# wh-xu/Hyper-Gen

Measured on AMD Instinct MI355X. Metric: genomes/sec sketch (k=21,s=1500,D=4096), higher is better.
Workload: dtype u64

## Files before the change

### hyper-gen_amd/__init__.py

```python
import ctypes as C
import os
import threading
import subprocess

import numpy as np

_HERE = os.path.dirname(os.path.abspath(__file__))
LIB_PATH = (os.environ.get("HYPERGEN_LIB") or None) or os.path.join(_HERE, "libhypergen_hip.so")
CLI_PATH = os.path.join(_HERE, "hyper-gen")

LAYOUT_SCALAR, LAYOUT_AVX2 = 0, 1
GATHER_PEER, GATHER_RCCL = 0, 1
ANI_MASH, ANI_CONTAINMENT, ANI_MAX_CONTAINMENT = 0, 1, 2
PAIRS_MASH, PAIRS_CONTAINMENT, PAIRS_MAX_CONTAINMENT, PAIRS_CONTAINMENT_REF = 1, 2, 4, 8
PAIRS_EMPTY = 0xFFFFFFFF
NORM_ACGT, NORM_U2T = 0, 1
(OK, ERR_INVALID, ERR_NO_DEVICE, ERR_HIP, ERR_OOM, ERR_CAPACITY, ERR_UNSUPPORTED, ERR_IO,
 ERR_INEXACT) = range(9)


T_NAMES = ("kmer", "sort", "encode", "dist_prep", "dist")
T_COUNT = len(T_NAMES)


# ... 5 lines not shown

class SketchParams(C.Structure):
    _fields_ = [("ksize", C.c_uint32), ("canonical", C.c_uint32), ("scaled", C.c_uint64),
                ("seed", C.c_uint64), ("hv_d", C.c_uint32), ("hv_layout", C.c_uint32),
                ("norm_mode", C.c_uint32), ("min_count", C.c_uint32)]


class AniHit(C.Structure):
    _fields_ = [("ref_idx", C.c_uint32), ("qry_idx", C.c_uint32), ("ani", C.c_float)]


ANI_HIT_DTYPE = np.dtype([("ref_idx", "<u4"), ("qry_idx", "<u4"), ("ani", "<f4")])
HAM_HIT_DTYPE = np.dtype([("ref_idx", "<u4"), ("qry_idx", "<u4"), ("dist", "<u4")])


class FileSketch(C.Structure):
    _fields_ = [("ksize", C.c_uint8), ("canonical", C.c_uint8), ("hv_quant_bits", C.c_uint8),
                ("pad", C.c_uint8), ("hv_norm_2", C.c_int32), ("scaled", C.c_uint64),
                ("seed", C.c_uint64), ("hv_d", C.c_uint64), ("file_str", C.c_char_p),
                ("hv", C.POINTER(C.c_int16)), ("hv_len", C.c_uint64)]


EXPORTS = [
    "hg_status_str", "hg_last_error", "hg_version", "hg_ctx_create", "hg_ctx_destroy",
    "hg_ctx_set_stream", "hg_ctx_reset_stream", "hg_ctx_sync", "hg_ctx_sketch_step_counts", "hg_sketch_plan_describe", "hg_logf_dev", "hg_ani_from_dots_dev", "hg_device_count", "hg_dev_alloc", "hg_dev_free",
    "hg_copy_h2d", "hg_copy_d2h", "hg_sketch_params_default", "hg_kmer_hash_sample",
    "hg_kmer_hash_sample_min_count",
    "hg_hv_encode", "hg_sketch_batch_dev", "hg_sketch_batch", "hg_dist_full", "hg_dist_full_dev",
    "hg_dist", "hg_dist_dev", "hg_sort_ani_hits", "hg_hv_quant_bits", "hg_hv_pack", "hg_hv_packed_bytes",
    "hg_hv_unpack", "hg_sketch_file_write", "hg_sketch_file_read", "hg_sketch_file_count",
    "hg_sketch_file_get", "hg_sketch_file_free", "hg_read_merge_seq", "hg_read_merge_seq_into", "hg_free",
    "hg_synth_genomes_dev", "hg_ctx_enable_timing", "hg_ctx_timings", "hg_ctx_last_kernel",
    "hg_hv_binarize_dev", "hg_hamming_full_dev", "hg_hamming_search_dev",
    "hg_ctx_set_debug", "hg_read_fastx_into", "hg_dist_block_dev", "hg_hamming_search_block_dev",
    "hg_multi_create", "hg_multi_destroy", "hg_multi_size", "hg_multi_ctx", "hg_multi_last_error", "hg_shard_range",
    "hg_multi_peer_report", "hg_multi_set_gather", "hg_multi_gather_mode", "hg_multi_gather_report",
    "hg_sketch_batch_multi", "hg_dist_multi", "hg_dist_multi_dev", "hg_hamming_search_multi",
    "hg_sort_ani_hits_dev", "hg_sort_ani_hits_staged", "hg_topk_per_query_dev", "hg_ctx_last_dist_path",
    "hg_ctx_last_hamming_path", "hg_read_fastx_pinned", "hg_pinned_free",
    "hg_sketch_stream_open", "hg_sketch_stream_push", "hg_sketch_stream_pop", "hg_sketch_stream_finish",
    "hg_sketch_stream_last_error", "hg_sketch_stream_close", "hg_sketch_stream_stats", "hg_device_numa_node", "hg_bind_thread_to_numa_node", "hg_dist_tile_order",
    "hg_sketch_stream_push_packed", "hg_pack2_size", "hg_pack2", "hg_unpack2_dev",
    "hg_sketch_stream_try_push", "hg_sketch_stream_max_pending",
    "hg_sketch_batch_dev_packed", "hg_pack2_batch_dev", "hg_pack2_dev",
    "hg_pack2s_size", "hg_pack2s", "hg_sketch_stream_push_packed_sparse",
    "hg_dist_ops_row_bytes", "hg_dist_ops_meta_bytes", "hg_dist_ops_padded_rows", "hg_dist_prep_ops_dev", "hg_dist_block_ops_dev",
    "hg_hv_packed_bytes_naive", "hg_hv_pack_naive", "hg_hv_unpack_naive", "hg_hv_payload_layout", "hg_hv_unpack_batch_dev",
    "hg_sketch_file_read_image", "hg_sketch_file_image", "hg_sketch_file_payload_offset",
    "hg_cluster_init_dev", "hg_cluster_add_hits_dev", "hg_cluster_finish_dev", "hg_cluster_dev", "hg_cluster",
    "hg_cluster_greedy_hits_dev", "hg_cluster_greedy_dev", "hg_cluster_greedy", "hg_ctx_cluster_greedy_rounds",
    "hg_cluster_setcover_hits_dev", "hg_cluster_setcover_dev", "hg_cluster_setcover", "hg_ctx_cluster_setcover_rounds",
    "hg_cluster_tree_hits_dev", "hg_cluster_tree_dev", "hg_cluster_tree", "hg_ctx_cluster_tree_rounds",
    "hg_cluster_average_matrix_dev", "hg_cluster_average_dev", "hg_cluster_average", "hg_ctx_cluster_average_rounds",
    "hg_cluster_complete_matrix_dev", "hg_cluster_complete_dev", "hg_cluster_complete", "hg_ctx_cluster_complete_rounds",
    "hg_cluster_stats_matrix_dev", "hg_cluster_stats_dev", "hg_cluster_stats",
    "hg_nj_matrix_dev", "hg_nj_dev", "hg_nj", "hg_nj_newick",
    "hg_ctx_set_ani_metric", "hg_ctx_ani_metric", "hg_multi_set_ani_metric",
    "hg_search_topk_dev", "hg_search_topk_block_dev", "hg_search_topk", "hg_search_topk_merge", "hg_search_topk_multi_dev",
    "hg_ani_pairs_dev", "hg_ani_pairs",
]
SEARCH_TOPK_MAX = 64
CLUSTER_AVERAGE_MAX_N = 65536
CLUSTER_COMPLETE_MAX_N = 65536
STATS_NONE = 0xFFFFFFFF
NJ_MAX_N = 65536
NJ_FRAC_BITS = 15
NJ_JOIN_DTYPE = np.dtype([("a", "<u4"), ("b", "<u4"), ("len_a", "<i8"), ("len_b", "<i8")])


class NodeStat(C.Structure):
    _fields_ = [("within_sum", C.c_uint64), ("within_min", C.c_uint32), ("within_min_idx", C.c_uint32),
                ("outside_max", C.c_uint32), ("outside_max_idx", C.c_uint32)]
# ... 67 lines not shown
        "hg_copy_d2h": (C.c_int, [vp, vp, vp, sz]),
        "hg_sketch_params_default": (None, [C.POINTER(SketchParams)]),
        "hg_kmer_hash_sample": (C.c_int, [vp, vp, sz, C.c_uint32, C.c_uint64, C.c_uint64, C.c_int,
                                          C.c_uint32, vp, sz, C.POINTER(sz)]),
        "hg_kmer_hash_sample_min_count": (C.c_int, [vp, vp, sz, C.c_uint32, C.c_uint64, C.c_uint64, C.c_int,
                                                    C.c_uint32, C.c_uint32, vp, sz, C.POINTER(sz)]),
        "hg_hv_encode": (C.c_int, [vp, vp, sz, C.c_uint32, C.c_uint32, vp, C.POINTER(C.c_int32)]),
        "hg_sketch_batch_dev": (C.c_int, [vp, vp, vp, vp, sz, C.POINTER(SketchParams), vp, vp, vp]),
        "hg_sketch_batch": (C.c_int, [vp, C.POINTER(vp), C.POINTER(sz), sz, C.POINTER(SketchParams),
                                      vp, vp, vp]),
        "hg_dist_full": (C.c_int, [vp, vp, vp, sz, vp, vp, sz, C.c_uint32, C.c_uint32, vp]),
        "hg_dist_full_dev": (C.c_int, [vp, vp, vp, sz, vp, vp, sz, C.c_uint32, C.c_uint32, vp]),
        "hg_ani_pairs_dev": (C.c_int, [vp, vp, vp, sz, vp, vp, sz, C.c_uint32, C.c_uint32, vp, sz, C.c_uint32, vp, vp]),
        "hg_ani_pairs": (C.c_int, [vp, vp, vp, sz, vp, vp, sz, C.c_uint32, C.c_uint32, vp, sz, C.c_uint32, vp, vp]),
        "hg_dist": (C.c_int, [vp, vp, vp, sz, vp, vp, sz, C.c_uint32, C.c_uint32, C.c_int, C.c_float,
                              vp, sz, C.POINTER(sz)]),
        "hg_dist_dev": (C.c_int, [vp, vp, vp, sz, vp, vp, sz, C.c_uint32, C.c_uint32, C.c_int,
                                  C.c_float, vp, sz, C.POINTER(sz)]),
        "hg_sort_ani_hits": (None, [vp, sz, sz, C.c_int]),
        "hg_hv_quant_bits": (C.c_uint32, [vp, C.c_uint32]),
        "hg_hv_pack": (C.c_int, [vp, C.c_uint32, C.c_uint32, vp]),
        "hg_hv_packed_bytes": (sz, [C.c_uint32, C.c_uint32]),
        "hg_hv_unpack": (C.c_int, [vp, C.c_uint32, C.c_uint32, vp]),
        "hg_sketch_file_write": (C.c_int, [C.c_char_p, C.POINTER(FileSketch), sz]),
        "hg_sketch_file_read": (C.c_int, [C.c_char_p, C.POINTER(vp)]),
        "hg_sketch_file_count": (sz, [vp]),
        "hg_sketch_file_get": (C.POINTER(FileSketch), [vp, sz]),
        "hg_sketch_file_free": (None, [vp]),
        "hg_read_merge_seq": (C.c_int, [C.c_char_p, C.POINTER(vp), C.POINTER(sz)]),
        "hg_read_merge_seq_into": (C.c_int, [C.c_char_p, C.POINTER(vp), C.POINTER(sz), C.POINTER(sz)]),
        "hg_read_fastx_into": (C.c_int, [C.c_char_p, C.c_uint32, C.POINTER(vp), C.POINTER(sz), C.POINTER(sz)]),
        "hg_ctx_set_debug": (C.c_int, [vp, C.c_char_p, C.c_char_p]),
        "hg_free": (None, [vp]),
        "hg_read_fastx_pinned": (C.c_int, [C.c_char_p, C.c_uint32, C.POINTER(vp), C.POINTER(sz), C.POINTER(sz)]),
        "hg_pinned_free": (None, [vp]),
        "hg_device_numa_node": (C.c_int, [C.c_int]),
        "hg_bind_thread_to_numa_node": (C.c_int, [C.c_int, C.c_uint]),
        "hg_dist_tile_order": (C.c_int, [C.c_uint32, C.c_uint32, C.c_uint32, C.c_uint32, C.c_int, C.c_int, C.c_uint64, C.c_uint64,
                                         C.c_void_p, C.c_size_t, C.POINTER(C.c_size_t)]),
        "hg_sketch_stream_open": (C.c_int, [C.POINTER(C.c_int), C.c_int, C.POINTER(SketchParams), C.POINTER(vp)]),
        "hg_sketch_stream_push": (C.c_int, [vp, vp, sz, C.c_uint64]),
        "hg_sketch_stream_pop": (C.c_int, [vp, C.POINTER(C.c_uint64), vp, C.POINTER(C.c_int32), C.POINTER(C.c_uint32),
                                           C.POINTER(C.c_int)]),
        "hg_sketch_stream_push_packed": (C.c_int, [vp, vp, sz, C.c_uint64]),
        "hg_sketch_stream_try_push": (C.c_int, [vp, vp, sz, C.c_uint64, C.c_int]),
        "hg_sketch_stream_max_pending": (sz, [vp]),
        "hg_pack2_size": (sz, [sz]),
        "hg_pack2": (C.c_int, [vp, sz, C.c_uint32, vp]),
        "hg_unpack2_dev": (C.c_int, [vp, vp, sz, vp]),
        "hg_sketch_batch_dev_packed": (C.c_int, [vp, vp, vp, vp, sz, C.POINTER(SketchParams), vp, vp, vp]),
        "hg_pack2_batch_dev": (C.c_int, [vp, vp, vp, vp, sz, C.c_uint32, vp, vp]),
        "hg_pack2_dev": (C.c_int, [vp, vp, sz, C.c_uint32, vp]),
        "hg_dist_ops_row_bytes": (sz, [C.c_uint32]),
        "hg_dist_ops_meta_bytes": (sz, []),
        "hg_dist_ops_padded_rows": (sz, [sz]),
        "hg_dist_prep_ops_dev": (C.c_int, [vp, vp, sz, C.c_uint32, vp, vp, vp]),
        "hg_dist_block_ops_dev": (C.c_int, [vp, vp, vp, vp, sz, sz, vp, vp, sz, vp, vp, sz, sz, C.c_uint32, C.c_uint32, C.c_int,
                                            C.c_float, vp, sz, C.POINTER(sz)]),
        "hg_pack2s_size": (sz, [sz, sz]),
        "hg_pack2s": (C.c_int, [vp, sz, C.c_uint32, vp, sz, C.POINTER(sz)]),
        "hg_sketch_stream_push_packed_sparse": (C.c_int, [vp, vp, sz, sz, C.c_uint64]),
        "hg_sketch_stream_finish": (C.c_int, [vp]),
        "hg_sketch_stream_last_error": (C.c_char_p, [vp]),
        "hg_sketch_stream_close": (None, [vp]),
        "hg_sketch_stream_stats": (C.c_int, [vp, C.c_int, C.POINTER(C.c_double)]),
        "hg_ctx_last_dist_path": (C.c_int, [vp]),
        "hg_ctx_set_ani_metric": (C.c_int, [vp, C.c_int]),
# ... 1257 lines not shown
```

### hyper-gen_amd/csrc/hg_api_sketch.hip

```cpp
#include <algorithm>
#include <atomic>
#include <cctype>
#include <chrono>
#include <cstdio>
#include <cstring>
#include <functional>
#include <memory>
#include <sched.h>
#include <string>
#include <thread>
#include <vector>

#include "hg_host.h"
#include "hg_hostfed_layout.h"

#include "hg_sketch.h"

static hg_status sketch_batch_dev_impl(hg_ctx *c, const uint8_t *d_seq, const uint64_t *offsets, const uint64_t *lens, size_t n,
                                       const hg_sketch_params *p, int16_t *d_hv, int32_t *d_norm2, uint32_t *d_nhash, bool packed,
                                       const uint64_t *mask_offs = nullptr) {
  if (!c) return HG_ERR_INVALID;
  hg_status s = hg_check_sketch_params(c, p);
  if (s != HG_OK) return s;
  if (n == 0) return HG_OK;
// ... 51 lines not shown
  if (((uintptr_t)d_seq & 3) || ((uintptr_t)d_blob & 15)) return hg_fail(c, HG_ERR_INVALID, "hg_pack2_dev: d_seq must be 4-byte, d_blob 16-byte aligned");
  const uint64_t zero = 0, len = n_bps;
  return hg_pack2_batch_dev(c, d_seq, &zero, &len, 1, norm_mode, d_blob, &zero);
}

extern "C" int hg_device_numa_node(int device_id) {
  char bus[64] = {0};
  if (hipDeviceGetPCIBusId(bus, (int)sizeof bus, device_id) != hipSuccess) return -1;
  for (char *q = bus; *q; ++q) *q = (char)std::tolower((unsigned char)*q);
  const std::string path = std::string("/sys/bus/pci/devices/") + bus + "/numa_node";
  FILE *f = std::fopen(path.c_str(), "r");
  if (!f) return -1;
  int node = -1;
  if (std::fscanf(f, "%d", &node) != 1) node = -1;
  std::fclose(f);
  return node;
}

namespace {
bool grow_pinned(uint8_t *&buf, size_t &cap, size_t need, size_t keep, void *) {
  if (need <= cap) return true;
  const size_t want = ((need + need / 8) + ((size_t)1 << 20) - 1) & ~(((size_t)1 << 20) - 1);
  void *nb = nullptr;
  if (hipHostMalloc(&nb, want, hipHostMallocPortable) != hipSuccess || !nb) return false;
  if (buf && keep) std::memcpy(nb, buf, std::min(keep, cap));
  if (buf) (void)hipHostFree(buf);
  buf = static_cast<uint8_t *>(nb), cap = want;
  return true;
}
}

extern "C" hg_status hg_read_fastx_pinned(const char *path, uint32_t mode, uint8_t **buf, size_t *cap, size_t *n_bps) {
  return hg_read_fastx_impl(path, mode, buf, cap, n_bps, grow_pinned, nullptr);
}

extern "C" void hg_pinned_free(void *p) {
  if (p) (void)hipHostFree(p);
}

static unsigned host_threads() {
  unsigned n = std::thread::hardware_concurrency();
  cpu_set_t set;
  if (sched_getaffinity(0, sizeof set, &set) == 0) n = std::min<unsigned>(n ? n : 1u, (unsigned)CPU_COUNT(&set));
  return std::max(1u, std::min(n, 16u));
}

static std::atomic<int> g_hostfed_calls{0};
namespace {
struct HostfedCall {
  int others;
  HostfedCall() : others(g_hostfed_calls.fetch_add(1)) {}
  ~HostfedCall() { g_hostfed_calls.fetch_sub(1); }
};
}
static bool host_pinned(const void *p) {
  hipPointerAttribute_t a;
  if (hipPointerGetAttributes(&a, p) != hipSuccess) {
    (void)hipGetLastError();
    return false;
  }
  return a.type == hipMemoryTypeHost;
}
namespace {
constexpr double HG_LINK_BYTES_PER_S = 50e9;
struct PackState {
  std::atomic<uint64_t> rate{0};
// ... 361 lines not shown
```

### hyper-gen_amd/csrc/hg_cli.cpp

```cpp
#include <fcntl.h>
#include <glob.h>
#include <sched.h>
#include <unistd.h>
#include <sys/stat.h>

#include <algorithm>
#include <atomic>
#include <bitset>
#include <cerrno>
#include <chrono>
#include <condition_variable>
#include <cstdarg>
#include <cstdio>
#include <cstdlib>
#include <cstring>
#include <ctime>
#include <deque>
#include <initializer_list>
#include <map>
#include <mutex>
#include <string>
#include <thread>
#include <utility>
#include <vector>

#include "../../include/hypergen.h"
#include "../../include/hypergen_aa.h"
#include "../../include/hypergen_tx.h"

namespace {

void logline(const char *lvl, const std::string &msg) {
  char ts[32];
  std::time_t t = std::time(nullptr);
  std::strftime(ts, sizeof ts, "%Y-%m-%d-%H:%M:%S", std::localtime(&t));
  std::printf("%s [%s] - %s\n", ts, lvl, msg.c_str());
  std::fflush(stdout);
}

bool debug_log() {
  static const bool on = [] {
    const char *e = std::getenv("RUST_LOG");
    return e && std::strstr(e, "debug") != nullptr;
  }();
  return on;
}
double now_s() { return std::chrono::duration<double>(std::chrono::steady_clock::now().time_since_epoch()).count(); }
void debugf(const char *fmt, ...) __attribute__((format(printf, 1, 2)));
void debugf(const char *fmt, ...) {
  if (!debug_log()) return;
  char buf[512];
  va_list ap;
  va_start(ap, fmt);
  std::vsnprintf(buf, sizeof buf, fmt, ap);
  va_end(ap);
  logline("DEBUG", buf);
}

[[noreturn]] void die(const std::string &msg) {
  std::fprintf(stderr, "error: %s\n", msg.c_str());
  std::fflush(nullptr);
  _exit(2);
}

enum class Linkage { single, greedy, setcover };
enum class SearchPath { automatic, hits, topk };
enum : unsigned { SKETCH = 1, DIST = 2, SEARCH = 4, CLUSTER = 8, ANY = 15 };

struct Cli {
  std::string mode, path = "1", path_r = "1", path_q = "1", out, method = "t1ha2", device = "cpu";
  unsigned mode_bit = 0;
  bool pack_naive = false;
  unsigned shards = 0;
  unsigned threads = 16, ksize = 21, top_n = 1;
  bool canonical = true;
  unsigned long long seed = 123, scaled = 1500, hv_d = 4096;
  float quant_scale = 1.0f, ani_th = 85.0f;
  bool protein = false;
  bool alphabet_given = false;
  bool translate = false;
// ... 378 lines not shown
}

void ck(hg_ctx *ctx, hg_status s, const char *what) {
  if (s != HG_OK) die(std::string(what) + ": " + hg_status_str(s) + " (" + hg_last_error(ctx) + ")");
}
void ckm(hg_multi *m, hg_status s, const char *what) {
  if (s != HG_OK) die(std::string(what) + ": " + hg_status_str(s) + " (" + hg_multi_last_error(m) + ")");
}

hg_multi *open_all_devices(unsigned shards) {
  const int n = hg_device_count();
  if (n <= 0) die(std::string("no MI355X device: ") + hg_last_error(nullptr));
  std::vector<int> ids(shards ? shards : (unsigned)n);
  for (size_t i = 0; i < ids.size(); ++i) ids[i] = (int)(i % (size_t)n);
  hg_multi *m = nullptr;
  if (hg_multi_create(ids.data(), (int)ids.size(), &m) != HG_OK) die(std::string("no MI355X device: ") + hg_last_error(nullptr));
  return m;
}

std::vector<std::string> fasta_files(const std::string &dir, std::initializer_list<const char *> patterns = {"*.fna", "*.fa", "*.fasta"}) {
  std::vector<std::string> out;
  for (const char *pat : patterns) {
    glob_t g;
    std::string p = dir + (dir.empty() || dir.back() == '/' ? "" : "/") + pat;
    if (glob(p.c_str(), 0, nullptr, &g) == 0)
      for (size_t i = 0; i < g.gl_pathc; ++i) out.push_back(g.gl_pathv[i]);
    globfree(&g);
  }
  return out;
}

int run_sketch_batches(const Cli &c, const std::vector<std::string> &files);

int run_sketch(const Cli &c) {
  if (c.path == "1" && c.out.empty()) die("the following required arguments were not provided: --path --out");
  if (c.out.empty()) die("the following required arguments were not provided: --out");
  if (c.protein) return run_sketch_batches(c, fasta_files(c.path, {"*.faa"}));
  if (c.translate) return run_sketch_batches(c, fasta_files(c.path));
  const auto files = fasta_files(c.path);
  const size_t n = files.size();
  logline("INFO", "Start sketching...");
  const double t0 = now_s();
  if (c.scaled == 0) die("scaled must be >= 1");
  if (c.hv_d == 0 || c.hv_d > 32768) die("hv_d must be in 1..32768");
  if (c.hv_d % 256)
    logline("WARN", "hv_d is not a multiple of 256: the dimensions behind the last whole block are lost in the .sketch file (as in the reference)");
  hg_sketch_params p;
  hg_sketch_params_default(&p);
  const bool gpu_mode = c.device == "gpu";
  p.ksize = c.ksize, p.scaled = c.scaled, p.seed = c.seed;
  p.canonical = gpu_mode ? (c.canonical ? 1u : 0u) : 1u;
  p.hv_d = (uint32_t)c.hv_d, p.hv_layout = HG_LAYOUT_AVX2;
  p.norm_mode = gpu_mode ? HG_NORM_ACGT : HG_NORM_U2T;
  p.min_count = c.min_count;
  const uint32_t read_mode = gpu_mode ? HG_READ_MERGE : HG_READ_NEEDLETAIL;

  std::vector<std::vector<int16_t>> payload(n);
  std::vector<hg_file_sketch> recs(n);

  const size_t T = std::max<size_t>(1, std::min<size_t>(c.threads, std::max<size_t>(n, 1)));
  const size_t S = std::max<size_t>(4, (64 + T - 1) / T);
  struct Slot {
    uint8_t *p = nullptr;
    size_t cap = 0, len = 0;
    bool busy = false;
  };
  std::vector<Slot> slots(T * S);
  std::vector<Slot *> slot_of(n, nullptr);
  std::mutex mu;
  std::condition_variable cv_stream;
  std::vector<std::condition_variable> cv_space(T);
  hg_sketch_stream *stream = nullptr;
  std::atomic<size_t> next{0};
  std::atomic<uint64_t> read_ns{0};
  std::vector<int> dev_node;
  std::atomic<size_t> n_packed{0};
  const uint32_t pack_flags = HG_READ_PACK2 | (p.norm_mode == HG_NORM_U2T ? HG_READ_PACK2_U2T : 0u);
  auto reader = [&](size_t tid) {
    (void)hg_bind_thread_to_numa_node(dev_node[tid % dev_node.size()], (unsigned)T);
    size_t k = 0;
    for (size_t i; (i = next.fetch_add(1)) < n; k = (k + 1) % S) {
      Slot &sl = slots[tid * S + k];
      bool pack;
      {
        std::unique_lock<std::mutex> lk(mu);
        size_t in_flight = 0;
        for (size_t q = 0; q < S; ++q) in_flight += slots[tid * S + q].busy ? 1 : 0;
        pack = in_flight >= 2;
        cv_space[tid].wait(lk, [&] { return !sl.busy; });
      }
      const double tr0 = now_s();
      if (hg_read_fastx_pinned(files[i].c_str(), read_mode | (pack ? pack_flags : 0u), &sl.p, &sl.cap, &sl.len) != HG_OK)
        die("Opening .fna files failed: " + files[i]);
      read_ns.fetch_add((uint64_t)((now_s() - tr0) * 1e9));
      if (pack) n_packed.fetch_add(1);
      {
        std::unique_lock<std::mutex> lk(mu);
        sl.busy = true, slot_of[i] = &sl;
        cv_stream.wait(lk, [&] { return stream != nullptr; });
      }
      const hg_status ps = pack ? hg_sketch_stream_push_packed(stream, sl.p, sl.len, i) : hg_sketch_stream_push(stream, sl.p, sl.len, i);
      if (ps != HG_OK) die(std::string("sketch: ") + hg_sketch_stream_last_error(stream));
    }
  };
  const double td0 = now_s();
  const int nd = hg_device_count();
  if (nd <= 0) die(std::string("no MI355X device: ") + hg_last_error(nullptr));
  for (int i = 0; i < nd; ++i) dev_node.push_back(hg_device_numa_node(i));
  std::vector<std::thread> readers;
  for (size_t t = 0; t < T && n; ++t) readers.emplace_back(reader, t);
  {
    std::vector<int> ids(nd);
    for (int i = 0; i < nd; ++i) ids[i] = i;
    hg_sketch_stream *st = nullptr;
    if (hg_sketch_stream_open(ids.data(), nd, &p, &st) != HG_OK) die(std::string("no MI355X device: ") + hg_last_error(nullptr));
    debugf("%d device(s) opened in %.1f ms", nd, (now_s() - td0) * 1e3);
    std::lock_guard<std::mutex> lk(mu);
    stream = st;
    cv_stream.notify_all();
  }
  std::vector<int16_t> hv(c.hv_d);
  double t_wait = 0, t_pack = 0;
  for (size_t done = 0; done < n; ++done) {
    uint64_t f = 0;
    int32_t n2 = 0;
    uint32_t nh = 0;
    int got = 0;
    const double tw0 = now_s();
    if (hg_sketch_stream_pop(stream, &f, hv.data(), &n2, &nh, &got) != HG_OK || !got)
      die(std::string("sketch: ") + hg_sketch_stream_last_error(stream));
    size_t owner;
    {
      std::lock_guard<std::mutex> lk(mu);
      slot_of[f]->busy = false;
      owner = (size_t)(slot_of[f] - slots.data()) / S;
    }
    cv_space[owner].notify_one();
    const double ts1 = now_s();
    const uint32_t q = hg_hv_quant_bits(hv.data(), (uint32_t)c.hv_d);
    const size_t pk_bytes = c.pack_naive ? hg_hv_packed_bytes_naive((uint32_t)c.hv_d, q) : hg_hv_packed_bytes((uint32_t)c.hv_d, q);
    payload[f].resize((pk_bytes + 1) / 2);
    if ((c.pack_naive ? hg_hv_pack_naive : hg_hv_pack)(hv.data(), (uint32_t)c.hv_d, q, reinterpret_cast<uint8_t *>(payload[f].data())) != HG_OK) die("pack");
    hg_file_sketch &r = recs[f];
    std::memset(&r, 0, sizeof r);
    r.ksize = (uint8_t)c.ksize, r.canonical = c.canonical, r.hv_quant_bits = (uint8_t)q, r.hv_norm_2 = n2;
    r.scaled = c.scaled, r.seed = c.seed, r.hv_d = c.hv_d;
    r.file_str = files[f].c_str();
    r.hv = payload[f].data(), r.hv_len = pk_bytes / 2;
    t_wait += ts1 - tw0, t_pack += now_s() - ts1;
  }
  for (auto &t : readers) t.join();
  if (debug_log()) {
    double st[6];
    for (int e = 0; hg_sketch_stream_stats(stream, e, st) == HG_OK; ++e)
      debugf("device engine %d: uploader idle %.1f ms, waiting for a chunk %.1f ms, in copy calls %.1f ms; compute idle "
             "%.1f ms, busy %.1f ms; %.0f chunks", e, st[0] * 1e3, st[1] * 1e3, st[2] * 1e3, st[3] * 1e3, st[4] * 1e3, st[5]);
  }
  debugf("collector: waited %.1f ms for results, sketch compression %.1f ms; readers: %.2f ms per file and thread, "
         "%zu of %zu files sent 2-bit packed", t_wait * 1e3, t_pack * 1e3, n ? read_ns.load() / 1e6 / n : 0.0,
         n_packed.load(), n);
  const double secs = now_s() - t0;
  char buf[256];
  std::snprintf(buf, sizeof buf, "Sketching %zu files took %.2fs - Speed: %.1f files/s", n, secs, n / std::max(secs, 1e-9));
  logline("INFO", buf);
  if (hg_sketch_file_write(c.out.c_str(), recs.data(), n) != HG_OK) die("Dump sketch file failed!");
  size_t total = 8;
  for (auto &r : recs) total += 47 + std::strlen(r.file_str) + r.hv_len * 2;
  std::snprintf(buf, sizeof buf, "Dump sketch file to %s with size %.2f MB", c.out.c_str(), total / 1024.0 / 1024.0);
  logline("INFO", buf);
  const double tf0 = now_s();
  hg_sketch_stream_close(stream);
  for (auto &sl : slots) hg_pinned_free(sl.p);
  debugf("released buffers and devices in %.1f ms", (now_s() - tf0) * 1e3);
  return 0;
}

template <class F>
void parallel(size_t n, F fn) {
  std::vector<std::thread> th;
  for (size_t t = 1; t < n; ++t) th.emplace_back([&fn, t] { fn(t); });
  fn(0);
  for (auto &t : th) t.join();
}

int run_sketch_batches(const Cli &c, const std::vector<std::string> &files) {
  const bool tx = c.translate;
  const uint32_t read_mode = c.device == "gpu" ? HG_READ_MERGE : HG_READ_NEEDLETAIL;
  const size_t n = files.size();
  logline("INFO", "Start sketching...");
  const double t0 = now_s();
  if (c.scaled == 0) die("scaled must be >= 1");
  if (c.hv_d == 0 || c.hv_d > 32768) die("hv_d must be in 1..32768");
  if (c.hv_d % 256)
    logline("WARN", "hv_d is not a multiple of 256: the dimensions behind the last whole block are lost in the .sketch file (as in the reference)");
  hg_sketch_params p;
  hg_sketch_params_default(&p);
  p.ksize = c.ksize, p.scaled = c.scaled, p.seed = c.seed, p.canonical = 0;
  p.hv_d = (uint32_t)c.hv_d, p.hv_layout = HG_LAYOUT_AVX2, p.norm_mode = HG_NORM_ACGT, p.min_count = 1;
  if (hg_device_count() <= 0) die(std::string("no MI355X device: ") + hg_last_error(nullptr));
  hg_ctx *ctx = nullptr;
  if (hg_ctx_create(0, &ctx) != HG_OK) die(std::string("no MI355X device: ") + hg_last_error(nullptr));

  std::vector<std::vector<int16_t>> payload(n);
  std::vector<hg_file_sketch> recs(n);
  constexpr size_t BATCH_FILES = 256, BATCH_BYTES = (size_t)1 << 30;
  struct Buf {
// ... 762 lines not shown
```

### hyper-gen_amd/csrc/hg_formats.cpp

```cpp
#include <fcntl.h>
#include <sched.h>
#include <sys/syscall.h>
#include <sys/stat.h>
#include <unistd.h>
#include <zlib.h>
#if defined(__x86_64__)
#include <immintrin.h>
#endif

#include <algorithm>
#include <cerrno>
#include <cstdio>
#include <cstdlib>
#include <cstring>
#include <new>
#include <string>
#include <vector>

#include "../../include/hypergen.h"
#include "hg_host.h"
#include "hg_pack2.h"

extern "C" uint32_t hg_hv_quant_bits(const int16_t *hv, uint32_t hv_d) {
  if (!hv || hv_d == 0) return 6;
// ... 687 lines not shown
    size_t n = 0;
    if (!grow(buf, cap, std::max(cap, ((size_t)16 << 20) + 64), 0, user)) st = HG_ERR_OOM;
    int got = 0;
    while (st == HG_OK && (got = gzread(f, buf + n, (unsigned)std::min<size_t>(cap - 64 - n, 1u << 30))) > 0) {
      n += (size_t)got;
      if (n == cap - 64 && !grow(buf, cap, 2 * cap, n, user)) st = HG_ERR_OOM;
    }
    if (st == HG_OK && got < 0) st = HG_ERR_IO;
    gzclose(f);
    *pbuf = buf, *pcap = cap;
    if (st != HG_OK) return st;
    NeedletailState gst;
    w = base_mode == HG_READ_NEEDLETAIL ? merge_lines_needletail(buf, n, buf, gst) : merge_lines(buf, n, buf);
    std::memset(buf + w, 0, 64);
    *n_bps = w;
    if (pack) return hg_pack2(buf, w, u2t ? HG_NORM_U2T : HG_NORM_ACGT, buf);
    return HG_OK;
  }
  *pbuf = buf, *pcap = cap;
  if (st != HG_OK) return st;
  if (pack) {
    pack2_span(mst.data(), have, u2t, buf + (w >> 2), mask + (w >> 3));
    w += have;
    pack2_finish(buf, w, mask);
  } else {
    std::memset(buf + w, 0, 64);
  }
  *n_bps = w;
  return HG_OK;
}

extern "C" hg_status hg_read_fastx_into(const char *path, uint32_t mode, uint8_t **pbuf, size_t *pcap, size_t *n_bps) {
  return hg_read_fastx_impl(path, mode, pbuf, pcap, n_bps, grow_malloc, nullptr);
}

extern "C" hg_status hg_read_merge_seq_into(const char *path, uint8_t **pbuf, size_t *pcap, size_t *n_bps) {
  return hg_read_fastx_into(path, HG_READ_MERGE, pbuf, pcap, n_bps);
}

extern "C" hg_status hg_read_merge_seq(const char *path, uint8_t **out, size_t *n_bps) {
  if (!path || !out || !n_bps) return HG_ERR_INVALID;
  *out = nullptr, *n_bps = 0;
  uint8_t *buf = nullptr;
  size_t cap = 0;
  const hg_status st = hg_read_merge_seq_into(path, &buf, &cap, n_bps);
  if (st != HG_OK) {
    std::free(buf);
    return st;
  }
  *out = buf;
  return HG_OK;
}

extern "C" void hg_free(void *p) { std::free(p); }

namespace {
void nj_put_length(std::string &w, int64_t len) {
  const unsigned __int128 mag = len < 0 ? (unsigned __int128)0 - (unsigned __int128)(__int128)len : (unsigned __int128)len;
  const unsigned __int128 t = (mag * 1000u + 16384u) >> 15;
  char buf[64];
  std::snprintf(buf, sizeof buf, "%s%llu.%08llu", len < 0 && t != 0 ? "-" : "", (unsigned long long)(t / 100000000u),
                (unsigned long long)(t % 100000000u));
  w += buf;
}
void nj_put_label(std::string &w, const char *name) {
  w += '\'';
// ... 90 lines not shown
```

### include/hypergen.h

```cpp
#ifndef HYPERGEN_H
#define HYPERGEN_H

#include <stddef.h>
#include <stdint.h>

#ifdef __cplusplus
extern "C" {
#endif

typedef struct hg_ctx hg_ctx;

typedef enum {
  HG_OK = 0,
  HG_ERR_INVALID = 1,
  HG_ERR_NO_DEVICE = 2,
  HG_ERR_HIP = 3,
  HG_ERR_OOM = 4,
  HG_ERR_CAPACITY = 5,
  HG_ERR_UNSUPPORTED = 6,
  HG_ERR_IO = 7,
  HG_ERR_INEXACT = 8
} hg_status;

const char *hg_status_str(hg_status s);
// ... 282 lines not shown
const hg_file_sketch *hg_sketch_file_get(const hg_sketch_file *f, size_t i);
void hg_sketch_file_free(hg_sketch_file *f);

typedef struct hg_sketch_stream hg_sketch_stream;
hg_status hg_sketch_stream_open(const int *device_ids, int n_devices, const hg_sketch_params *p, hg_sketch_stream **out);
hg_status hg_sketch_stream_push(hg_sketch_stream *s, const uint8_t *seq, size_t n_bps, uint64_t tag);
hg_status hg_sketch_stream_push_packed(hg_sketch_stream *s, const uint8_t *blob, size_t n_bps, uint64_t tag);
hg_status hg_sketch_stream_push_packed_sparse(hg_sketch_stream *s, const uint8_t *blob, size_t blob_bytes, size_t n_bps, uint64_t tag);
hg_status hg_sketch_stream_try_push(hg_sketch_stream *s, const uint8_t *data, size_t n_bps, uint64_t tag, int packed);
size_t hg_sketch_stream_max_pending(const hg_sketch_stream *s);
hg_status hg_sketch_stream_pop(hg_sketch_stream *s, uint64_t *tag, int16_t *hv_out, int32_t *norm2_out,
                               uint32_t *nhash_out, int *got);
hg_status hg_sketch_stream_finish(hg_sketch_stream *s);
const char *hg_sketch_stream_last_error(hg_sketch_stream *s);
hg_status hg_sketch_stream_stats(hg_sketch_stream *s, int engine, double out[6]);
void hg_sketch_stream_close(hg_sketch_stream *s);

size_t hg_pack2_size(size_t n_bps);
hg_status hg_pack2(const uint8_t *seq, size_t n_bps, uint32_t norm_mode, uint8_t *out);
hg_status hg_unpack2_dev(hg_ctx *ctx, const uint8_t *d_blob, size_t n_bps, uint8_t *d_seq_out);
size_t hg_pack2s_size(size_t n_bps, size_t n_runs);
hg_status hg_pack2s(const uint8_t *seq, size_t n_bps, uint32_t norm_mode, uint8_t *out, size_t cap, size_t *size_out);
hg_status hg_pack2_batch_dev(hg_ctx *ctx, const uint8_t *d_seq, const uint64_t *offsets, const uint64_t *lens, size_t n,
                             uint32_t norm_mode, uint8_t *d_blobs, const uint64_t *blob_offsets);
hg_status hg_pack2_dev(hg_ctx *ctx, const uint8_t *d_seq, size_t n_bps, uint32_t norm_mode, uint8_t *d_blob);

hg_status hg_read_merge_seq(const char *path, uint8_t **out, size_t *n_bps);
hg_status hg_read_merge_seq_into(const char *path, uint8_t **buf, size_t *cap, size_t *n_bps);
#define HG_READ_MERGE 0u
#define HG_READ_NEEDLETAIL 1u
#define HG_READ_PACK2 16u
#define HG_READ_PACK2_U2T 32u
hg_status hg_read_fastx_into(const char *path, uint32_t mode, uint8_t **buf, size_t *cap, size_t *n_bps);
hg_status hg_read_fastx_pinned(const char *path, uint32_t mode, uint8_t **buf, size_t *cap, size_t *n_bps);
void hg_pinned_free(void *p);
hg_status hg_dist_tile_order(uint32_t tiles_m, uint32_t tiles_n, uint32_t tile_rows, uint32_t tile_cols, int diagonal_first,
                             int symmetric, uint64_t ref_off, uint64_t qry_off, uint32_t *out, size_t cap, size_t *n_slots);
int hg_device_numa_node(int device_id);
int hg_bind_thread_to_numa_node(int node, unsigned threads_sharing);
void hg_free(void *p);

typedef struct {
  uint32_t ref_idx;
  uint32_t qry_idx;
  uint32_t dist;
} hg_ham_hit;
hg_status hg_hv_binarize_dev(hg_ctx *ctx, const int16_t *d_hv, size_t n, uint32_t hv_d, uint32_t *d_bits);
hg_status hg_hamming_full_dev(hg_ctx *ctx, const uint32_t *d_ref_bits, size_t R, const uint32_t *d_qry_bits,
                              size_t Q, uint32_t hv_d, uint32_t *d_dist_out);
hg_status hg_hamming_search_dev(hg_ctx *ctx, const uint32_t *d_ref_bits, size_t R, const uint32_t *d_qry_bits,
                                size_t Q, uint32_t hv_d, uint32_t max_dist, hg_ham_hit *d_out, size_t cap,
                                size_t *n_out);

int hg_ctx_last_hamming_path(const hg_ctx *ctx);
hg_status hg_hamming_search_block_dev(hg_ctx *ctx, const uint32_t *d_ref_bits, size_t R, size_t ref_off,
                                      const uint32_t *d_qry_bits, size_t Q, size_t qry_off, uint32_t hv_d,
                                      uint32_t max_dist, hg_ham_hit *d_out, size_t cap, size_t *n_out);

typedef struct hg_multi hg_multi;
hg_status hg_multi_create(const int *device_ids, int n, hg_multi **out);
void hg_multi_destroy(hg_multi *m);
int hg_multi_size(const hg_multi *m);
hg_ctx *hg_multi_ctx(hg_multi *m, int shard);
const char *hg_multi_last_error(const hg_multi *m);
const char *hg_multi_peer_report(const hg_multi *m);
enum { HG_GATHER_PEER = 0, HG_GATHER_RCCL = 1 };
hg_status hg_multi_set_gather(hg_multi *m, int mode);
// ... 35 lines not shown
```

Before: 129,300.

## Overlap HIP device open with file listing and read-ahead, skip teardown on exit

Moves HIP runtime init and sketch-stream opening onto a separate thread so directory listing and FASTA reading start at once. Readers can optionally pre-read and pack files into a huge-page mmap arena before the stream exists, then copy them into pinned slots. The process also exits via _exit without freeing device and pinned resources unless HYPER_GEN_TEARDOWN is set. This is meant to hide startup and shutdown latency in end-to-end time, at the cost of extra host copies and skipped cleanup.

```diff
diff --git a/hyper-gen_amd/__init__.py b/hyper-gen_amd/__init__.py
--- a/hyper-gen_amd/__init__.py
+++ b/hyper-gen_amd/__init__.py
@@ -61,12 +61,12 @@
     "hg_sketch_file_get", "hg_sketch_file_free", "hg_read_merge_seq", "hg_read_merge_seq_into", "hg_free",
     "hg_synth_genomes_dev", "hg_ctx_enable_timing", "hg_ctx_timings", "hg_ctx_last_kernel",
     "hg_hv_binarize_dev", "hg_hamming_full_dev", "hg_hamming_search_dev",
-    "hg_ctx_set_debug", "hg_read_fastx_into", "hg_dist_block_dev", "hg_hamming_search_block_dev",
+    "hg_ctx_set_debug", "hg_read_fastx_into", "hg_read_fastx_fixed", "hg_dist_block_dev", "hg_hamming_search_block_dev",
     "hg_multi_create", "hg_multi_destroy", "hg_multi_size", "hg_multi_ctx", "hg_multi_last_error", "hg_shard_range",
     "hg_multi_peer_report", "hg_multi_set_gather", "hg_multi_gather_mode", "hg_multi_gather_report",
     "hg_sketch_batch_multi", "hg_dist_multi", "hg_dist_multi_dev", "hg_hamming_search_multi",
     "hg_sort_ani_hits_dev", "hg_sort_ani_hits_staged", "hg_topk_per_query_dev", "hg_ctx_last_dist_path",
-    "hg_ctx_last_hamming_path", "hg_read_fastx_pinned", "hg_pinned_free",
+    "hg_ctx_last_hamming_path", "hg_read_fastx_pinned", "hg_pinned_reserve", "hg_pinned_free",
     "hg_sketch_stream_open", "hg_sketch_stream_push", "hg_sketch_stream_pop", "hg_sketch_stream_finish",
     "hg_sketch_stream_last_error", "hg_sketch_stream_close", "hg_sketch_stream_stats", "hg_device_numa_node", "hg_bind_thread_to_numa_node", "hg_dist_tile_order",
     "hg_sketch_stream_push_packed", "hg_pack2_size", "hg_pack2", "hg_unpack2_dev",
@@ -200,7 +200,9 @@
         "hg_read_fastx_into": (C.c_int, [C.c_char_p, C.c_uint32, C.POINTER(vp), C.POINTER(sz), C.POINTER(sz)]),
         "hg_ctx_set_debug": (C.c_int, [vp, C.c_char_p, C.c_char_p]),
         "hg_free": (None, [vp]),
+        "hg_read_fastx_fixed": (C.c_int, [C.c_char_p, C.c_uint32, vp, sz, C.POINTER(sz)]),
         "hg_read_fastx_pinned": (C.c_int, [C.c_char_p, C.c_uint32, C.POINTER(vp), C.POINTER(sz), C.POINTER(sz)]),
+        "hg_pinned_reserve": (C.c_int, [C.POINTER(vp), C.POINTER(sz), sz]),
         "hg_pinned_free": (None, [vp]),
         "hg_device_numa_node": (C.c_int, [C.c_int]),
         "hg_bind_thread_to_numa_node": (C.c_int, [C.c_int, C.c_uint]),
diff --git a/hyper-gen_amd/csrc/hg_api_sketch.hip b/hyper-gen_amd/csrc/hg_api_sketch.hip
--- a/hyper-gen_amd/csrc/hg_api_sketch.hip
+++ b/hyper-gen_amd/csrc/hg_api_sketch.hip
@@ -107,6 +107,15 @@
 
 extern "C" hg_status hg_read_fastx_pinned(const char *path, uint32_t mode, uint8_t **buf, size_t *cap, size_t *n_bps) {
   return hg_read_fastx_impl(path, mode, buf, cap, n_bps, grow_pinned, nullptr);
+}
+
+extern "C" hg_status hg_pinned_reserve(uint8_t **buf, size_t *cap, size_t need) {
+  if (!buf || !cap) return HG_ERR_INVALID;
+  uint8_t *b = *buf;
+  size_t c = b ? *cap : 0;
+  const bool ok = grow_pinned(b, c, need, 0, nullptr);
+  *buf = b, *cap = c;
+  return ok ? HG_OK : HG_ERR_OOM;
 }
 
 extern "C" void hg_pinned_free(void *p) {
diff --git a/hyper-gen_amd/csrc/hg_cli.cpp b/hyper-gen_amd/csrc/hg_cli.cpp
--- a/hyper-gen_amd/csrc/hg_cli.cpp
+++ b/hyper-gen_amd/csrc/hg_cli.cpp
@@ -2,6 +2,7 @@
 #include <glob.h>
 #include <sched.h>
 #include <unistd.h>
+#include <sys/mman.h>
 #include <sys/stat.h>
 
 #include <algorithm>
@@ -46,6 +47,8 @@
   return on;
 }
 double now_s() { return std::chrono::duration<double>(std::chrono::steady_clock::now().time_since_epoch()).count(); }
+const double t_entry = now_s();
+double since_entry_ms() { return (now_s() - t_entry) * 1e3; }
 void debugf(const char *fmt, ...) __attribute__((format(printf, 1, 2)));
 void debugf(const char *fmt, ...) {
   if (!debug_log()) return;
@@ -490,19 +493,32 @@
 
 int run_sketch_batches(const Cli &c, const std::vector<std::string> &files);
 
+size_t read_ahead_budget() {
+  size_t budget = 0;
+  if (const char *e = std::getenv("HYPER_GEN_READ_AHEAD")) {
+    char *end = nullptr;
+    const unsigned long long v = std::strtoull(e, &end, 10);
+    if (*e && !*end) budget = (size_t)v;
+  }
+  if (!budget) return 0;
+  if (FILE *f = std::fopen("/proc/meminfo", "r")) {
+    char line[128];
+    unsigned long long kb = 0;
+    while (std::fgets(line, sizeof line, f))
+      if (std::sscanf(line, "MemAvailable: %llu kB", &kb) == 1) budget = std::min(budget, (size_t)kb * 1024 / 4);
+    std::fclose(f);
+  }
+  return budget;
+}
+
 int run_sketch(const Cli &c) {
   if (c.path == "1" && c.out.empty()) die("the following required arguments were not provided: --path --out");
   if (c.out.empty()) die("the following required arguments were not provided: --out");
   if (c.protein) return run_sketch_batches(c, fasta_files(c.path, {"*.faa"}));
   if (c.translate) return run_sketch_batches(c, fasta_files(c.path));
-  const auto files = fasta_files(c.path);
-  const size_t n = files.size();
-  logline("INFO", "Start sketching...");
-  const double t0 = now_s();
+  debugf("options parsed %.1f ms after process entry", since_entry_ms());
   if (c.scaled == 0) die("scaled must be >= 1");
   if (c.hv_d == 0 || c.hv_d > 32768) die("hv_d must be in 1..32768");
-  if (c.hv_d % 256)
-    logline("WARN", "hv_d is not a multiple of 256: the dimensions behind the last whole block are lost in the .sketch file (as in the reference)");
   hg_sketch_params p;
   hg_sketch_params_default(&p);
   const bool gpu_mode = c.device == "gpu";
@@ -513,6 +529,42 @@
   p.min_count = c.min_count;
   const uint32_t read_mode = gpu_mode ? HG_READ_MERGE : HG_READ_NEEDLETAIL;
 
+  std::mutex mu;
+  std::condition_variable cv_stream;
+  std::atomic<bool> runtime_up{false};
+  std::atomic<hg_sketch_stream *> stream{nullptr};
+  std::vector<int> dev_node;
+  const double td0 = now_s();
+  std::thread opener([&] {
+    const int nd = hg_device_count();
+    if (nd <= 0) die(std::string("no MI355X device: ") + hg_last_error(nullptr));
+    std::vector<int> ids(nd), nodes(nd);
+    for (int i = 0; i < nd; ++i) ids[i] = i, nodes[i] = hg_device_numa_node(i);
+    debugf("HIP runtime up in %.1f ms", (now_s() - td0) * 1e3);
+    {
+      std::lock_guard<std::mutex> lk(mu);
+      dev_node = nodes;
+      runtime_up = true;
+    }
+    cv_stream.notify_all();
+    hg_sketch_stream *st = nullptr;
+    if (hg_sketch_stream_open(ids.data(), nd, &p, &st) != HG_OK) die(std::string("no MI355X device: ") + hg_last_error(nullptr));
+    debugf("%d device(s) opened in %.1f ms", nd, (now_s() - td0) * 1e3);
+    {
+      std::lock_guard<std::mutex> lk(mu);
+      stream = st;
+    }
+    cv_stream.notify_all();
+  });
+
+  const auto files = fasta_files(c.path);
+  const size_t n = files.size();
+  debugf("directory listed (%zu files) %.1f ms after process entry", n, since_entry_ms());
+  logline("INFO", "Start sketching...");
+  const double t0 = now_s();
+  if (c.hv_d % 256)
+    logline("WARN", "hv_d is not a multiple of 256: the dimensions behind the last whole block are lost in the .sketch file (as in the reference)");
+
   std::vector<std::vector<int16_t>> payload(n);
   std::vector<hg_file_sketch> recs(n);
 
@@ -523,60 +575,123 @@
     size_t cap = 0, len = 0;
     bool busy = false;
   };
+  struct Ahead {
+    uint8_t *p = nullptr;
+    size_t n_bps = 0, bytes = 0, file = 0;
+  };
   std::vector<Slot> slots(T * S);
   std::vector<Slot *> slot_of(n, nullptr);
-  std::mutex mu;
-  std::condition_variable cv_stream;
   std::vector<std::condition_variable> cv_space(T);
-  hg_sketch_stream *stream = nullptr;
   std::atomic<size_t> next{0};
   std::atomic<uint64_t> read_ns{0};
-  std::vector<int> dev_node;
+  const size_t budget = read_ahead_budget();
+  std::atomic<size_t> ahead_files{0}, ahead_total{0};
+  std::atomic<bool> pushed{false};
+  constexpr size_t ARENA_BLOCK = (size_t)64 << 20, HUGE = (size_t)2 << 20;
+  std::vector<std::pair<void *, size_t>> arena_blocks;
+  size_t first_files = 0, first_bytes = 0;
+  double first_push_ms = 0;
   std::atomic<size_t> n_packed{0};
   const uint32_t pack_flags = HG_READ_PACK2 | (p.norm_mode == HG_NORM_U2T ? HG_READ_PACK2_U2T : 0u);
   auto reader = [&](size_t tid) {
-    (void)hg_bind_thread_to_numa_node(dev_node[tid % dev_node.size()], (unsigned)T);
-    size_t k = 0;
-    for (size_t i; (i = next.fetch_add(1)) < n; k = (k + 1) % S) {
-      Slot &sl = slots[tid * S + k];
-      bool pack;
-      {
+    bool bound = false;
+    auto bind = [&] {
+      if (bound || !runtime_up.load()) return;
+      (void)hg_bind_thread_to_numa_node(dev_node[tid % dev_node.size()], (unsigned)T);
+      bound = true;
+    };
+    auto wait_runtime = [&] {
+      if (!runtime_up.load()) {
         std::unique_lock<std::mutex> lk(mu);
-        size_t in_flight = 0;
-        for (size_t q = 0; q < S; ++q) in_flight += slots[tid * S + q].busy ? 1 : 0;
-        pack = in_flight >= 2;
-        cv_space[tid].wait(lk, [&] { return !sl.busy; });
+        cv_stream.wait(lk, [&] { return runtime_up.load(); });
       }
-      const double tr0 = now_s();
-      if (hg_read_fastx_pinned(files[i].c_str(), read_mode | (pack ? pack_flags : 0u), &sl.p, &sl.cap, &sl.len) != HG_OK)
-        die("Opening .fna files failed: " + files[i]);
-      read_ns.fetch_add((uint64_t)((now_s() - tr0) * 1e9));
-      if (pack) n_packed.fetch_add(1);
+      bind();
+    };
+    auto wait_slot = [&](Slot &sl) {
+      std::unique_lock<std::mutex> lk(mu);
+      size_t in_flight = 0;
+      for (size_t q = 0; q < S; ++q) in_flight += slots[tid * S + q].busy ? 1 : 0;
+      cv_space[tid].wait(lk, [&] { return !sl.busy; });
+      return in_flight >= 2;
+    };
+    auto push = [&](Slot &sl, bool pack, size_t i) {
+      hg_sketch_stream *st = nullptr;
       {
         std::unique_lock<std::mutex> lk(mu);
         sl.busy = true, slot_of[i] = &sl;
-        cv_stream.wait(lk, [&] { return stream != nullptr; });
+        cv_stream.wait(lk, [&] { return (st = stream.load()) != nullptr; });
       }
-      const hg_status ps = pack ? hg_sketch_stream_push_packed(stream, sl.p, sl.len, i) : hg_sketch_stream_push(stream, sl.p, sl.len, i);
-      if (ps != HG_OK) die(std::string("sketch: ") + hg_sketch_stream_last_error(stream));
+      if (!pushed.exchange(true)) first_files = ahead_files.load(), first_bytes = ahead_total.load(), first_push_ms = since_entry_ms();
+      const hg_status ps = pack ? hg_sketch_stream_push_packed(st, sl.p, sl.len, i) : hg_sketch_stream_push(st, sl.p, sl.len, i);
+      if (ps != HG_OK) die(std::string("sketch: ") + hg_sketch_stream_last_error(st));
+    };
+    size_t k = 0;
+    std::deque<Ahead> ahead;
+    uint8_t *arena = nullptr;
+    size_t arena_left = 0;
+    auto arena_room = [&](size_t need) {
+      if (arena_left >= need) return true;
+      const size_t sz = std::max(ARENA_BLOCK, (need + HUGE - 1) & ~(HUGE - 1));
+      void *m = mmap(nullptr, sz + HUGE, PROT_READ | PROT_WRITE, MAP_PRIVATE | MAP_ANONYMOUS | MAP_NORESERVE, -1, 0);
+      if (m == MAP_FAILED) return false;
+      arena = reinterpret_cast<uint8_t *>(((uintptr_t)m + HUGE - 1) & ~(uintptr_t)(HUGE - 1)), arena_left = sz;
+      (void)madvise(arena, sz, MADV_HUGEPAGE);
+      std::lock_guard<std::mutex> lk(mu);
+      arena_blocks.emplace_back(m, sz + HUGE);
+      return true;
+    };
+    auto drain = [&] {
+      for (; !ahead.empty(); ahead.pop_front(), k = (k + 1) % S) {
+        const Ahead &a = ahead.front();
+        Slot &sl = slots[tid * S + k];
+        (void)wait_slot(sl);
+        if (hg_pinned_reserve(&sl.p, &sl.cap, a.bytes + 64) != HG_OK) die("sketch: out of page-locked memory");
+        std::memcpy(sl.p, a.p, a.bytes);
+        sl.len = a.n_bps;
+        push(sl, true, a.file);
+      }
+    };
+    for (size_t i; (i = next.fetch_add(1)) < n;) {
+      bind();
+      const double tr0 = now_s();
+      struct stat sb;
+      if (!stream.load() && ahead_total.load() < budget &&
+          arena_room((::stat(files[i].c_str(), &sb) == 0 ? (size_t)sb.st_size : 0) + 4096)) {
+        Ahead a;
+        const hg_status rs = hg_read_fastx_fixed(files[i].c_str(), read_mode | pack_flags, arena, arena_left, &a.n_bps);
+        if (rs == HG_OK) {
+          read_ns.fetch_add((uint64_t)((now_s() - tr0) * 1e9));
+          a.p = arena, a.bytes = hg_pack2_size(a.n_bps), a.file = i;
+          const size_t took = std::min(arena_left, (a.bytes + 64 + 4095) & ~(size_t)4095);
+          arena += took, arena_left -= took;
+          ahead_total.fetch_add(a.bytes), ahead_files.fetch_add(1), n_packed.fetch_add(1);
+          ahead.push_back(a);
+          continue;
+        }
+        if (rs != HG_ERR_OOM) die("Opening .fna files failed: " + files[i]);
+      }
+      wait_runtime();
+      drain();
+      Slot &sl = slots[tid * S + k];
+      const bool pack = wait_slot(sl);
+      const double tr1 = now_s();
+      if (hg_read_fastx_pinned(files[i].c_str(), read_mode | (pack ? pack_flags : 0u), &sl.p, &sl.cap, &sl.len) != HG_OK)
+        die("Opening .fna files failed: " + files[i]);
+      read_ns.fetch_add((uint64_t)((now_s() - tr1) * 1e9));
+      if (pack) n_packed.fetch_add(1);
+      push(sl, pack, i);
+      k = (k + 1) % S;
+    }
+    if (!ahead.empty()) {
+      wait_runtime();
+      drain();
     }
   };
-  const double td0 = now_s();
-  const int nd = hg_device_count();
-  if (nd <= 0) die(std::string("no MI355X device: ") + hg_last_error(nullptr));
-  for (int i = 0; i < nd; ++i) dev_node.push_back(hg_device_numa_node(i));
   std::vector<std::thread> readers;
   for (size_t t = 0; t < T && n; ++t) readers.emplace_back(reader, t);
-  {
-    std::vector<int> ids(nd);
-    for (int i = 0; i < nd; ++i) ids[i] = i;
-    hg_sketch_stream *st = nullptr;
-    if (hg_sketch_stream_open(ids.data(), nd, &p, &st) != HG_OK) die(std::string("no MI355X device: ") + hg_last_error(nullptr));
-    debugf("%d device(s) opened in %.1f ms", nd, (now_s() - td0) * 1e3);
-    std::lock_guard<std::mutex> lk(mu);
-    stream = st;
-    cv_stream.notify_all();
-  }
+  opener.join();
+  hg_sketch_stream *const open_stream = stream.load();
+  debugf("stream open %.1f ms after process entry", since_entry_ms());
   std::vector<int16_t> hv(c.hv_d);
   double t_wait = 0, t_pack = 0;
   for (size_t done = 0; done < n; ++done) {
@@ -585,8 +700,8 @@
     uint32_t nh = 0;
     int got = 0;
     const double tw0 = now_s();
-    if (hg_sketch_stream_pop(stream, &f, hv.data(), &n2, &nh, &got) != HG_OK || !got)
-      die(std::string("sketch: ") + hg_sketch_stream_last_error(stream));
+    if (hg_sketch_stream_pop(open_stream, &f, hv.data(), &n2, &nh, &got) != HG_OK || !got)
+      die(std::string("sketch: ") + hg_sketch_stream_last_error(open_stream));
     size_t owner;
     {
       std::lock_guard<std::mutex> lk(mu);
@@ -608,9 +723,12 @@
     t_wait += ts1 - tw0, t_pack += now_s() - ts1;
   }
   for (auto &t : readers) t.join();
+  debugf("first push %.1f ms, last result %.1f ms after process entry", first_push_ms, since_entry_ms());
+  debugf("read ahead of the stream: %zu files, %.1f MB packed, before the first push (%zu files, %.1f MB in all; budget %.0f MB)",
+         first_files, first_bytes / 1e6, ahead_files.load(), ahead_total.load() / 1e6, budget / 1e6);
   if (debug_log()) {
     double st[6];
-    for (int e = 0; hg_sketch_stream_stats(stream, e, st) == HG_OK; ++e)
+    for (int e = 0; hg_sketch_stream_stats(open_stream, e, st) == HG_OK; ++e)
       debugf("device engine %d: uploader idle %.1f ms, waiting for a chunk %.1f ms, in copy calls %.1f ms; compute idle "
              "%.1f ms, busy %.1f ms; %.0f chunks", e, st[0] * 1e3, st[1] * 1e3, st[2] * 1e3, st[3] * 1e3, st[4] * 1e3, st[5]);
   }
@@ -627,9 +745,17 @@
   std::snprintf(buf, sizeof buf, "Dump sketch file to %s with size %.2f MB", c.out.c_str(), total / 1024.0 / 1024.0);
   logline("INFO", buf);
   const double tf0 = now_s();
-  hg_sketch_stream_close(stream);
+  debugf("sketch file written %.1f ms after process entry", since_entry_ms());
+  if (!std::getenv("HYPER_GEN_TEARDOWN")) {
+    debugf("leaving without teardown %.1f ms after process entry", since_entry_ms());
+    std::fflush(nullptr);
+    _exit(0);
+  }
+  hg_sketch_stream_close(open_stream);
   for (auto &sl : slots) hg_pinned_free(sl.p);
+  for (auto &b : arena_blocks) (void)munmap(b.first, b.second);
   debugf("released buffers and devices in %.1f ms", (now_s() - tf0) * 1e3);
+  debugf("leaving main %.1f ms after process entry", since_entry_ms());
   return 0;
 }
 
diff --git a/hyper-gen_amd/csrc/hg_formats.cpp b/hyper-gen_amd/csrc/hg_formats.cpp
--- a/hyper-gen_amd/csrc/hg_formats.cpp
+++ b/hyper-gen_amd/csrc/hg_formats.cpp
@@ -743,6 +743,12 @@
 
 extern "C" hg_status hg_read_fastx_into(const char *path, uint32_t mode, uint8_t **pbuf, size_t *pcap, size_t *n_bps) {
   return hg_read_fastx_impl(path, mode, pbuf, pcap, n_bps, grow_malloc, nullptr);
+}
+
+extern "C" hg_status hg_read_fastx_fixed(const char *path, uint32_t mode, uint8_t *buf, size_t cap, size_t *n_bps) {
+  if (!buf) return HG_ERR_INVALID;
+  return hg_read_fastx_impl(path, mode, &buf, &cap, n_bps,
+                            [](uint8_t *&, size_t &have, size_t need, size_t, void *) { return need <= have; }, nullptr);
 }
 
 extern "C" hg_status hg_read_merge_seq_into(const char *path, uint8_t **pbuf, size_t *pcap, size_t *n_bps) {
diff --git a/include/hypergen.h b/include/hypergen.h
--- a/include/hypergen.h
+++ b/include/hypergen.h
@@ -338,7 +338,9 @@
 #define HG_READ_PACK2 16u
 #define HG_READ_PACK2_U2T 32u
 hg_status hg_read_fastx_into(const char *path, uint32_t mode, uint8_t **buf, size_t *cap, size_t *n_bps);
+hg_status hg_read_fastx_fixed(const char *path, uint32_t mode, uint8_t *buf, size_t cap, size_t *n_bps);
 hg_status hg_read_fastx_pinned(const char *path, uint32_t mode, uint8_t **buf, size_t *cap, size_t *n_bps);
+hg_status hg_pinned_reserve(uint8_t **buf, size_t *cap, size_t need);
 void hg_pinned_free(void *p);
 hg_status hg_dist_tile_order(uint32_t tiles_m, uint32_t tiles_n, uint32_t tile_rows, uint32_t tile_cols, int diagonal_first,
                              int symmetric, uint64_t ref_off, uint64_t qry_off, uint32_t *out, size_t cap, size_t *n_slots);
```

Result: no change. 129,400, median of 2 (+0.1%).
